# loro-dev/loro

Hardware: NVIDIA H100
Metric: merged CRDT ops/sec (batched docs) (higher is better)
Workload: dtype int64

## Files before the change

loro_b200/csrc/engine.cu:

```cuda
#include "../../include/loro_b200.h"

#include <algorithm>
#include <atomic>
#include <chrono>
#include <memory>
#include <mutex>
#include <string>
#include <thread>
#include <unordered_map>
#include <vector>
#include <cstring>
#include <cstdio>
#include <cstdlib>
#include <sched.h>

#include "lb_defs.h"
#include "k_frame.cuh"
#include "k_decode.cuh"
#include "k_decode_warp.cuh"
#include "k_resolve.cuh"
#include "k_classify.cuh"
#include "k_checkout.cuh"
#include "k_seq.cuh"
#include "k_tree.cuh"
// ... 322 lines not shown
struct DocsetBlob { std::shared_ptr<DocsetBuf> buf; u64 off; u32 len; };
struct DocsetDoc { std::vector<DocsetBlob> blobs; };
struct lb_docset {
    int device = 0;
    std::mutex mu;
    std::unordered_map<u64, DocsetDoc> docs;
    u64 stored_bytes = 0;
};

struct lb_exports {
    struct Answer { lb_status status; const char* error; const uint8_t* bytes; size_t len; };
    std::vector<Answer> answers;
    std::vector<std::unique_ptr<uint8_t[]>> bufs;
};

namespace {

const int TPB = 128;
inline unsigned nblk(u64 n, int tpb = TPB) { return (unsigned)((n + tpb - 1) / tpb); }

#define LB_BATCH_LAUNCH(b, kernel, grid, block, smem, ...)                          \
    do {                                                                            \
        LB_LAUNCH(kernel, grid, block, smem, (b)->dev.stream, __VA_ARGS__);         \
        (b)->timings.kernel_launches++;                                             \
    } while (0)

u32* BatchTables::* const SG_TABLES[] = {
    &BatchTables::sg_src, &BatchTables::sg_r0, &BatchTables::sg_from, &BatchTables::sg_atoms, &BatchTables::sg_est,
    &BatchTables::sg_nmops, &BatchTables::sg_ndel, &BatchTables::sg_nrows, &BatchTables::sg_last_head, &BatchTables::sg_skip};
u32* BatchTables::* const FC_TABLES[] = {
    &BatchTables::fc_src, &BatchTables::fc_pos, &BatchTables::fc_r0, &BatchTables::fc_from, &BatchTables::fc_atoms,
    &BatchTables::fc_nrows, &BatchTables::fc_ndel, &BatchTables::fc_skip, &BatchTables::fc_tail, &BatchTables::fc_est};

void launch_exp_encode(lb_batch* b, u64 NOB, const BatchTables& xt, XBlock* xb, u32* xscratch, u8* out, int retry, bool cuts) {
    if (!NOB) return;
    const bool capped = NOB >= LB_XENC_BOUNDED_MIN_BLOCKS;
    if (cuts && capped) LB_BATCH_LAUNCH(b, k_exp_encode_cut<1>, nblk(NOB, 64), 64, 0, b->d_docs, NOB, xt, xb, xscratch, out, retry);
    else if (cuts) LB_BATCH_LAUNCH(b, k_exp_encode_cut<0>, nblk(NOB, 64), 64, 0, b->d_docs, NOB, xt, xb, xscratch, out, retry);
    else if (capped) LB_BATCH_LAUNCH(b, k_exp_encode<1>, nblk(NOB, 64), 64, 0, b->d_docs, NOB, xt, xb, xscratch, out, retry);
    else LB_BATCH_LAUNCH(b, k_exp_encode<0>, nblk(NOB, 64), 64, 0, b->d_docs, NOB, xt, xb, xscratch, out, retry);
}

unsigned seq_resident_ctas(int device) {
#ifdef LB_SIMT_EMU
    (void)device;
    return 1;
#else
    static std::atomic<unsigned> ctas[64];
    std::atomic<unsigned>& n = ctas[(unsigned)device % 64];
    if (!n.load(std::memory_order_relaxed)) {
        int per_sm = 0, sms = 0;
        CK(cudaOccupancyMaxActiveBlocksPerMultiprocessor(&per_sm, k_seq_integrate<1>, 32 * LB_SEQ_WARPS, 0));
        CK(cudaDeviceGetAttribute(&sms, cudaDevAttrMultiProcessorCount, device));
        if (per_sm < 1 || sms < 1) {
            g_last_error = "k_seq_integrate: no CTA fits a multiprocessor";
            throw lb_status(LB_ERR_CUDA);
        }
        n.store((unsigned)per_sm * (unsigned)sms, std::memory_order_relaxed);
    }
    return n.load(std::memory_order_relaxed);
#endif
}

void trace_point(lb_batch* b, const char* name);
void mark(lb_batch* b, BatchEvent e) {
    CK(cudaEventRecord(b->ev[e], b->dev.stream));
    b->ev_recorded[e] = true;
}

template <class T>
T d2h_one(lb_batch* b, const T* src) {
    T v;
    CK(cudaMemcpyAsync(&v, src, sizeof(T), cudaMemcpyDeviceToHost, b->dev.stream));
// ... 1433 lines not shown
```

loro_b200/csrc/k_export.cuh:

```cuda
#pragma once
#include "lb_tables.cuh"

enum { XK_NONE = 0, XK_LIST = 1, XK_TEXT = 2, XK_DEL = 3, XK_MAPSET = 4, XK_MAPDEL = 5, XK_TREE = 6 };
#define LB_MAX_BLOCK_SIZE 4096
#define XF_HEAD 1u
#define XF_SEG 2u

struct XDoc {
    u32 n_fc, n_mb;
    u32 flags;
    u32 n_prank;
    u64 ob0;
    u64 scratch0;
    u64 exp_off;
    u32 exp_len;
    u32 scratch_words;
    u64 stage0;
    u64 ovf0;
    u64 restage0;
};
struct XBlock {
    u32 doc;
    u32 fc0, fc1;
    u32 len;
    u32 sec_len[8];
    u32 col_len[9];
    u64 off;
    u64 scratch;
    u32 n_rows, n_dels;
    u32 n_ops, n_del_ops, n_pos;
    u64 stage;
    u32 stage_cap;
    u32 ovf;
};

struct XSink {
    u8* dst;
    u64 n, cap;
    __device__ __forceinline__ XSink(u8* d, u64 c) : dst(d), n(0), cap(c) {}
    __device__ __forceinline__ void put(u8 c) { if (n < cap) dst[n] = c; n++; }
    __device__ __forceinline__ void varint(u64 v) { while (v >= 0x80) { put((u8)(v | 0x80)); v >>= 7; } put((u8)v); }
    __device__ __forceinline__ void zigzag(i64 v) { varint(((u64)v << 1) ^ (u64)(v >> 63)); }
    __device__ __forceinline__ void copy(const u8* s, u64 len) {
        if (n + len <= cap) {
            u8* d = dst + n;
            u64 i = 0;
            while (i < len && ((uintptr_t)(d + i) & 3)) { d[i] = s[i]; i++; }
            for (; i + 4 <= len; i += 4) {
                u32 w = (u32)s[i] | ((u32)s[i + 1] << 8) | ((u32)s[i + 2] << 16) | ((u32)s[i + 3] << 24);
                *(u32*)(d + i) = w;
            }
            for (; i < len; i++) d[i] = s[i];
        }
        n += len;
    }
};
__device__ __forceinline__ u32 varint_len(u64 v) { u32 k = 1; while (v >= 0x80) { v >>= 7; k++; } return k; }

struct XOp {
    u8 xk; u32 cidx; i32 ctr; u32 atoms; i32 prop; u32 f0, f1; i32 f2; u32 st0, nst;
    u32 g;
};
__device__ __forceinline__ u32 xop_estimate(const XOp& o) {
    switch (o.xk) {
        case XK_LIST: return 4 * o.atoms;
        case XK_TEXT: return o.f1 - o.f0;
        case XK_DEL: return 8;
        case XK_TREE: return 8;
        default: return 3;
    }
}
__device__ __forceinline__ u32 str_gen(u32 end) {
    u32 k = 0;
    u64 cap = 32;
    while (cap < end) { cap <<= 1; k++; }
    return k;
}
__device__ __forceinline__ bool d_bidi(const XOp& o) { return o.f2 == 1 || o.f2 == -1; }
__device__ __forceinline__ i64 d_start_pos(const XOp& o) { return o.f2 > 0 ? o.prop : (i64)o.prop + 1 + o.f2; }
__device__ __forceinline__ i64 d_next_pos(const XOp& o) { return o.f2 > 0 ? d_start_pos(o) : d_start_pos(o) - 1; }
__device__ __forceinline__ i64 d_prev_pos(const XOp& o) { return o.f2 > 0 ? o.prop : (i64)o.prop + 1; }
__device__ __forceinline__ i64 d_id_end(const XOp& o) { return (i64)(i32)o.f1 + (o.f2 < 0 ? -o.f2 : o.f2); }
__device__ inline bool xop_mergable(const XOp& a, const XOp& b) {
    if (a.ctr + (i32)a.atoms != b.ctr || a.cidx != b.cidx || a.xk != b.xk) return false;
    switch (a.xk) {
        case XK_LIST: return (i64)a.prop + a.atoms == b.prop && a.f1 == b.f0;
        case XK_TEXT: return (i64)a.prop + a.atoms == b.prop && a.f1 == b.f0 && a.g == b.g;
// ... 439 lines not shown

struct XEntry {
    u32 src, from;
    u32 pos, r0;
    u32 atoms, est_ops, nmops, ndel, nrows;
    u32 skip;
    u32 tail;
    u32 lh_ch, lh_row;
    XOp last;
    bool last_valid;
};
struct XStore {
    bool have_block, open_valid, open_starts_block;
    u32 blk_est;
    XEntry open;
    XOp back;
};
__device__ __forceinline__ bool xmsg_same(const BatchTables& t, u32 a, u32 b) {
    u32 la = t.ch_msg_len[a], lb = t.ch_msg_len[b];
    if (la != lb) return false;
    const u8* pa = t.bytes + t.ch_msg_off[a];
    const u8* pb = t.bytes + t.ch_msg_off[b];
    for (u32 i = 0; i < la; i++)
        if (pa[i] != pb[i]) return false;
    return true;
}
__device__ __forceinline__ u32 xentry_ndeps(const BatchTables& t, const XEntry& e) {
    return e.from ? 1u : t.ch_ndeps[e.src] + (t.ch_dep_self[e.src] ? 1u : 0u);
}
struct XRows {
    const BatchTables& t; u32 pos; u32 r; u32 ch; u32 nr; u64 row0;
    u32 skip;
    __device__ XRows(const BatchTables& t_, u32 pos_, u32 r_) : t(t_), pos(pos_), r(r_), skip(0) { load(); }
    __device__ void load() { ch = t.ch_aorder[pos]; change_rows(t, ch, &row0, &nr); }
    __device__ u64 row() const { return row0 + r; }
    __device__ void next() {
        r++;
        skip = 0;
        while (r >= nr) {
            pos++; r = 0; ch = t.ch_aorder[pos];
            if (!t.ch_applied[ch]) { nr = 0; continue; }
            change_rows(t, ch, &row0, &nr);
            if (t.ch_trim[ch]) { r = t.sg_r0[ch]; skip = t.sg_skip[ch]; }
        }
    }
};
__device__ inline XOp xop_gather(const BatchTables& t, const DocInfo& di, XRows& it, u32& left, u32 skip = 0, u32 tail = 0) {
    XOp o = xop_from_row(t, di, it.ch, it.row());
    if (skip) xop_slice_front(t, o, it.row(), skip);
    left--;
    if (left) it.next();
    while (left && !(xr_flag(t, it.row()) & XF_HEAD)) {
        XOp x = xop_from_row(t, di, it.ch, it.row());
        if (it.skip) xop_slice_front(t, x, it.row(), it.skip);
        xop_merge(o, x);
        left--;
        if (left) it.next();
    }
    if (!left && tail) xop_slice_back(t, o, it.row(), tail);
    return o;
}
__device__ inline XOp xentry_last_op(const BatchTables& t, const DocInfo& di, const XEntry& E) {
    if (E.last_valid) return E.last;
    u64 row0;
    u32 nr;
    change_rows(t, E.lh_ch, &row0, &nr);
// ... 363 lines not shown
    {
        i64 prev_delta = 0;
        for (u32 i = 1; i < n; i++) {
            i64 dl = val(i) - val(i - 1);
            i64 x = dl - prev_delta;
            prev_delta = dl;
            if (x == 0) total_bits += 1;
            else if (x >= -63 && x <= 64) total_bits += 9;
            else if (x >= -255 && x <= 256) total_bits += 12;
            else if (x >= -2047 && x <= 2048) total_bits += 16;
            else if (x >= -1048575 && x <= 1048576) total_bits += 26;
            else total_bits += 69;
        }
    }
    int used = (int)(total_bits & 7);
    s.put((u8)(used == 0 ? 8 : used));
    XBits bw(s);
    i64 prev_delta = 0;
    for (u32 i = 1; i < n; i++) {
        i64 dl = val(i) - val(i - 1);
        i64 x = dl - prev_delta;
        prev_delta = dl;
        if (x == 0) bw.bit(false);
        else if (x >= -63 && x <= 64) { bw.bits(2, 2); bw.bits((u64)(x + 63), 7); }
        else if (x >= -255 && x <= 256) { bw.bits(6, 3); bw.bits((u64)(x + 255), 9); }
        else if (x >= -2047 && x <= 2048) { bw.bits(14, 4); bw.bits((u64)(x + 2047), 12); }
        else if (x >= -1048575 && x <= 1048576) { bw.bits(30, 5); bw.bits((u64)(x + 1048575), 21); }
        else { bw.bits(31, 5); bw.bits((u64)x, 64); }
    }
    if (bw.nbits) s.put((u8)((bw.cur & 0xFF) << (8 - bw.nbits)));
}

struct XReg {
    u32* ord; u32* inv; u32 n;
    __device__ u32 reg(u32 v) {
        if (inv[v] != 0xFFFFFFFFu) return inv[v];
        inv[v] = n;
        ord[n] = v;
        return n++;
    }
};
__device__ inline void xvalue_copy(XSink& s, const u8* p, u32 n, const BatchTables& t, u64 src_key0, XReg& keys) {
    Cur c(p, n);
    u32 stack[24];
    int sp = 0;
    while (!c.err) {
        while (sp > 0 && (stack[sp - 1] & 0x7fffffffu) == 0) sp--;
        if (sp == 0 && c.empty()) return;
        if (sp > 0) {
            stack[sp - 1]--;
            if (stack[sp - 1] & 0x80000000u) {
                u32 dk = t.key_map[src_key0 + (u32)c.varint()];
                s.varint(keys.reg(dk));
            }
        }
        u8 kind = c.get();
        s.put(kind);
        switch (kind) {
            case 0: case 1: case 2: break;
            case 3: { const u8* a = c.p; (void)c.sleb(); s.copy(a, (u64)(c.p - a)); break; }
            case 4: { const u8* a = c.p; c.skip(8); s.copy(a, (u64)(c.p - a)); break; }
            case 5: case 6: { const u8* a = c.p; u64 l = c.varint(); c.skip(l); s.copy(a, (u64)(c.p - a)); break; }
            case 7: case 8: {
                u64 cnt = c.varint();
                s.varint(cnt);
                if (sp >= 24 || cnt > (1u << 28)) return;
                stack[sp++] = (u32)cnt | (kind == 8 ? 0x80000000u : 0u);
                break;
            }
            case 9: s.put(c.get()); break;
            default: return;
        }
    }
// ... 40 lines not shown
    const DocInfo& di = docs[d];
    if (di.code != DOC_OK || !di.has_tree) return;
    const u64 p_lo = t.blocks[di.b0].pos0;
    const u32 n = (u32)(t.blocks[di.b1].pos0 - p_lo);
    u64* key = t.ps_key + p_lo;
    u32* val = t.ps_val + p_lo;
    for (u32 i = lane; i < n; i += 32) {
        const u8* pb = t.pos_pool + t.pos_off[p_lo + i];
        u32 pl = t.pos_len[p_lo + i];
        u64 k = 0;
        for (u32 q = 0; q < 8; q++) k = (k << 8) | (q < pl ? pb[q] : 0u);
        if (k == ~0ull) k--;
        key[i] = k;
        val[i] = i;
    }
    __syncwarp();
    warp_sort_pairs(key, val, n, lane, [&](u32 a, u32 b) -> bool { return xpos_cmp(t, (u32)p_lo + a, (u32)p_lo + b) < 0; });
    u32 carry = 0;
    for (u32 j0 = 0; j0 < n; j0 += 32) {
        u32 j = j0 + (u32)lane;
        int fresh = 0;
        if (j < n) fresh = (j == 0 || xpos_cmp(t, (u32)p_lo + val[j - 1], (u32)p_lo + val[j]) != 0) ? 1 : 0;
        int incl = warp_incl_scan(fresh, lane);
        if (j < n) {
            u32 rank = carry + (u32)incl - 1;
            t.pos_rank[p_lo + val[j]] = rank;
            if (fresh) t.pos_rep[p_lo + rank] = (u32)p_lo + val[j];
        }
        carry += (u32)__shfl_sync(LB_FULL, incl, 31);
    }
    if (lane == 0) t.xdoc[d].n_prank = carry;
}

#define LB_XENC_BOUNDED_MIN_BLOCKS 100000ull
template <int CUT>
__device__ __forceinline__ void exp_encode_body(
    const DocInfo* __restrict__ docs, u64 n_blocks, const BatchTables& t, XBlock* __restrict__ xb,
                             u32* __restrict__ scratch, u8* __restrict__ out, int retry) {
    u64 bi_ = (u64)blockIdx.x * blockDim.x + threadIdx.x;
    if (bi_ >= n_blocks) return;
    XBlock B = xb[bi_];
    if (retry) {
        if (!B.ovf) return;
        out += t.xdoc[B.doc].restage0;
    }
    const DocInfo& di = docs[B.doc];
    const u32 P = di.P, K = di.K, C = di.C;
    u32* sc = scratch + B.scratch;
    XReg peers, keys, cids;
    peers.ord = sc; peers.inv = sc + P;
    keys.ord = sc + 2 * P; keys.inv = keys.ord + K;
    cids.ord = keys.ord + 2 * K; cids.inv = cids.ord + C;
    u32* c_cidx = cids.ord + 2 * C;
    u32* c_prop = c_cidx + B.n_rows;
    u32* c_vt = c_prop + B.n_rows;
    u32* c_atoms = c_vt + B.n_rows;
    u32* d_peer = c_atoms + B.n_rows;
    u32* d_ctr = d_peer + B.n_dels;
    u32* d_len = d_ctr + B.n_dels;
    const bool has_tree = (t.xdoc[B.doc].flags & 2u) != 0;
    const bool has_maps = (t.xdoc[B.doc].flags & 4u) != 0;
    u32* p_rank = d_len + B.n_dels;
    const u64 pos_lo = has_tree ? t.blocks[di.b0].pos0 : 0;
    auto pos_local = [&](u32 gpos) -> u32 {
        u32 r = t.pos_rank[gpos];
        u32 lo = 0, hi = B.n_pos;
        while (lo < hi) { u32 mid = (lo + hi) >> 1; if (p_rank[mid] < r) lo = mid + 1; else hi = mid; }
        return lo;
    };
    auto w_tree_value = [&](XSink& s, u32 ti) {
        uint4 ids = t.tr_ids[ti];
        u32 pk = ids.z & 3u;
        s.varint(peers.inv[ids.x]);
        s.varint(ids.y);
        s.varint(pk == TRP_DELETED ? 0u : pos_local(t.tr_pos[ti]));
        s.put(pk == TRP_ROOT ? 1 : 0);
        if (pk != TRP_ROOT) { s.varint(peers.inv[ids.z >> 2]); s.varint(ids.w); }
    };
    const u32 fc0 = B.fc0, N = B.fc1 - B.fc0;
    const u32 first_src = t.fc_src[fc0];
    u32 n_dep = 0;
    for (u32 j = 0; j < N; j++) n_dep += t.fc_from[fc0 + j] ? 0u : t.ch_ndeps[t.fc_src[fc0 + j]];
    for (u32 i = 0; i < P; i++) peers.inv[i] = 0xFFFFFFFFu;
    for (u32 i = 0; i < K; i++) keys.inv[i] = 0xFFFFFFFFu;
    for (u32 i = 0; i < C; i++) cids.inv[i] = 0xFFFFFFFFu;
    peers.n = keys.n = cids.n = 0;
    peers.reg(t.peer_map[t.blocks[t.ch_block[first_src]].peer0]);
    B.n_pos = 0;
    if (has_tree) {
        u32 m = 0;
        for (u32 j = 0; j < N; j++) {
            XRows it(t, t.fc_pos[fc0 + j], t.fc_r0[fc0 + j]);
            u32 left = t.fc_nrows[fc0 + j];
            while (left) {
                uint4 r = xr_rec(t, it.row());
                if ((r.x & 7u) == XK_TREE && t.tr_pos[r.w] != 0xFFFFFFFFu) p_rank[m++] = t.pos_rank[t.tr_pos[r.w]];
                left--;
                if (left) it.next();
            }
        }
        auto sift = [&](u32 root, u32 end) {
            while (true) {
                u32 c = 2 * root + 1;
                if (c >= end) break;
                if (c + 1 < end && p_rank[c + 1] > p_rank[c]) c++;
                if (p_rank[root] >= p_rank[c]) break;
                u32 tmp = p_rank[root]; p_rank[root] = p_rank[c]; p_rank[c] = tmp;
                root = c;
            }
        };
        for (u32 i = m / 2; i-- > 0;) sift(i, m);
        for (u32 e = m; e-- > 1;) { u32 tmp = p_rank[0]; p_rank[0] = p_rank[e]; p_rank[e] = tmp; sift(0, e); }
        u32 w = 0;
        for (u32 i = 0; i < m; i++) if (i == 0 || p_rank[i] != p_rank[w - 1]) p_rank[w++] = p_rank[i];
        B.n_pos = w;
    }
    XSink vs(out + B.stage, B.stage_cap);
    u32 n_ops = 0, n_del = 0;
    u32 prev_cidx = 0, prev_prop = 0, prev_dp = 0, prev_dc = 0, prev_dl = 0;
    for (u32 j = 0; j < N; j++) {
        XRows it(t, t.fc_pos[fc0 + j], t.fc_r0[fc0 + j]);
        u32 left = t.fc_nrows[fc0 + j];
        u32 skip = t.fc_skip[fc0 + j];
        while (left) {
            XRows it0 = it;
            const u32 left0 = left;
            const u32 skip0 = skip;
            XOp o = xop_gather(t, di, it, left, skip);
            if (CUT && !left) xop_slice_back(t, o, it.row(), t.fc_tail[fc0 + j]);
            skip = left ? it.skip : 0u;
            if (o.xk == XK_LIST) { vs.put(7); vs.varint(o.atoms); }
            else if (o.xk == XK_TEXT) vs.varint(o.f1 - o.f0);
            u32 lc = cids.reg(o.cidx);
            u32 lp = (o.xk == XK_MAPSET || o.xk == XK_MAPDEL) ? keys.reg((u32)o.prop) : (u32)o.prop;
            if (o.xk == XK_LIST || o.xk == XK_TEXT || o.xk == XK_MAPSET) {
                u32 k = left0 - left;
                while (k) {
                    const u8* pp;
                    u32 pn;
                    const u32 sk = k == left0 - left ? skip0 : it0.skip;
                    xr_payload_skip(t, it0.row(), o.xk, sk, &pp, &pn);
                    if (CUT && k == 1 && !left && t.fc_tail[fc0 + j]) xr_payload_drop_tail(o.xk, xr_len(t, it0.row()) - sk, t.fc_tail[fc0 + j], pp, &pn);
                    if (has_maps && o.xk != XK_TEXT) xvalue_copy(vs, pp, pn, t, t.blocks[t.ch_block[it0.ch]].key0, keys);
                    else vs.copy(pp, pn);
                    k--;
                    if (k) it0.next();
                }
            }
            c_cidx[n_ops] = lc - prev_cidx; prev_cidx = lc;
            c_prop[n_ops] = lp - prev_prop; prev_prop = lp;
            c_vt[n_ops] = xk_value_type(o.xk);
            c_atoms[n_ops] = o.atoms;
            if (o.xk == XK_TREE) {
                uint4 ids = t.tr_ids[o.f0];
                peers.reg(ids.x);
                if ((ids.z & 3u) != TRP_ROOT) peers.reg(ids.z >> 2);
                w_tree_value(vs, o.f0);
            }
            if (o.xk == XK_DEL) {
                u32 dp = peers.reg(o.f0);
                d_peer[n_del] = dp - prev_dp; prev_dp = dp;
                d_ctr[n_del] = o.f1 - prev_dc; prev_dc = o.f1;
                d_len[n_del] = (u32)o.f2 - prev_dl; prev_dl = (u32)o.f2;
                n_del++;
            }
            n_ops++;
        }
    }
    B.n_ops = n_ops;
    B.n_del_ops = n_del;
    B.sec_len[7] = (u32)vs.n;
    for (u32 i = 0; i < cids.n; i++) {
        const DocContainer& dc = t.dcont[di.cid0 + cids.ord[i]];
        if (dc.is_root) keys.reg(dc.key_or_peer); else peers.reg(dc.key_or_peer);
    }
    for (u32 j = 0; j < N; j++) {
        if (t.fc_from[fc0 + j]) continue;
        u32 src = t.fc_src[fc0 + j];
        const BlockInfo& sb = t.blocks[t.ch_block[src]];
        for (u32 k = 0; k < t.ch_ndeps[src]; k++) peers.reg(t.peer_map[sb.peer0 + t.dep_peer_idx[t.ch_dep0[src] + k]]);
    }

    auto dep_self = [&](u32 j) -> bool { return t.fc_from[fc0 + j] ? true : t.ch_dep_self[t.fc_src[fc0 + j]] != 0; };
    auto dep_local = [&](XDeps& dc, u32 i) -> i64 {
        u64 di_ = dc.at(i);
        const BlockInfo& sb = t.blocks[t.ch_block[t.fc_src[fc0 + dc.j]]];
        return (i64)peers.inv[t.peer_map[sb.peer0 + t.dep_peer_idx[di_]]];
    };
    auto lamport = [&](u32 j) -> i64 { return (i64)t.ch_lamport[t.fc_src[fc0 + j]] + t.fc_from[fc0 + j]; };
    auto w_header = [&](XSink& s) {
        s.varint(peers.n);
        for (u32 i = 0; i < peers.n; i++) {
            u64 id = t.dpeer[di.peer0 + peers.ord[i]].id;
            for (int k = 0; k < 8; k++) s.put((u8)(id >> (8 * k)));
        }
        for (u32 j = 0; j + 1 < N; j++) s.varint(t.fc_atoms[fc0 + j]);
        enc_boolrle(s, N, dep_self);
        { XDeps dc(t, fc0, N); enc_anyrle(s, N, [&](u32 j) -> i64 { return (i64)dc.nd(j); }, WrVarint()); }
        { XDeps dc(t, fc0, N); enc_anyrle(s, n_dep, [&](u32 i) -> i64 { return dep_local(dc, i); }, WrVarint()); }
        { XDeps dc(t, fc0, N); enc_dod(s, n_dep, [&](u32 i) -> i64 { return (i64)t.dep_counter[dc.at(i)]; }); }
        enc_dod(s, N - 1, lamport);
    };
    auto w_meta = [&](XSink& s) {
        enc_dod(s, N, [&](u32 j) -> i64 { return t.ch_ts[t.fc_src[fc0 + j]]; });
        enc_anyrle(s, N, [&](u32 j) -> i64 { return (i64)t.ch_msg_len[t.fc_src[fc0 + j]]; }, WrVarint());
        for (u32 j = 0; j < N; j++) {
            u32 src = t.fc_src[fc0 + j];
            s.copy(t.bytes + t.ch_msg_off[src], t.ch_msg_len[src]);
        }
    };
    auto w_cids = [&](XSink& s) {
        s.varint(cids.n);
        for (u32 i = 0; i < cids.n; i++) {
            const DocContainer& dc = t.dcont[di.cid0 + cids.ord[i]];
            s.varint(4);
            s.put(dc.is_root ? 1 : 0);
            s.put(dc.type);
            if (dc.is_root) { s.varint(0); s.zigzag((i64)keys.inv[dc.key_or_peer]); }
            else { s.varint(peers.inv[dc.key_or_peer]); s.zigzag((i64)dc.counter); }
        }
    };
    auto w_keys = [&](XSink& s) {
        for (u32 i = 0; i < keys.n; i++) {
            u32 k = keys.ord[i];
            s.varint(t.dkey_len[di.key0 + k]);
            s.copy(t.bytes + t.dkey_off[di.key0 + k], t.dkey_len[di.key0 + k]);
        }
    };
    auto w_opcol = [&](XSink& s, int col) {
        switch (col) {
            case 0: enc_anyrle(s, n_ops, [&](u32 i) -> i64 { return (i64)(i32)c_cidx[i]; }, WrZigzag()); break;
            case 1: enc_anyrle(s, n_ops, [&](u32 i) -> i64 { return (i64)(i32)c_prop[i]; }, WrZigzag()); break;
            case 2: enc_anyrle(s, n_ops, [&](u32 i) -> i64 { return (i64)c_vt[i]; }, WrByte()); break;
            default: enc_anyrle(s, n_ops, [&](u32 i) -> i64 { return (i64)c_atoms[i]; }, WrVarint());
        }
    };
    auto w_delcol = [&](XSink& s, int col) {
        switch (col) {
            case 0: enc_anyrle(s, n_del, [&](u32 i) -> i64 { return (i64)(i32)d_peer[i]; }, WrZigzag()); break;
            case 1: enc_anyrle(s, n_del, [&](u32 i) -> i64 { return (i64)(i32)d_ctr[i]; }, WrZigzag()); break;
            default: enc_anyrle(s, n_del, [&](u32 i) -> i64 { return (i64)(i32)d_len[i]; }, WrZigzag());
        }
    };
    auto pos_bytes_of = [&](u32 i, const u8** pb) -> u32 { u32 g = t.pos_rep[pos_lo + p_rank[i]]; *pb = t.pos_pool + t.pos_off[g]; return t.pos_len[g]; };
    auto pos_common = [&](u32 i) -> u32 {
        if (i == 0) return 0;
        const u8 *a, *b;
        u32 la = pos_bytes_of(i - 1, &a), lb = pos_bytes_of(i, &b);
        u32 n = la < lb ? la : lb, k = 0;
        while (k < n && a[k] == b[k]) k++;
        return k;
    };
    auto w_poscol = [&](XSink& s, int col) {
        if (col == 0) enc_anyrle(s, B.n_pos, [&](u32 i) -> i64 { return (i64)pos_common(i); }, WrVarint());
        else {
            s.varint(B.n_pos);
            for (u32 i = 0; i < B.n_pos; i++) {
                const u8* pb;
                u32 pl = pos_bytes_of(i, &pb), c = pos_common(i);
                s.varint(pl - c);
                s.copy(pb + c, pl - c);
            }
        }
    };
    u32 counter_len = 0;
    for (u32 j = 0; j < N; j++) counter_len += t.fc_atoms[fc0 + j];
    u32 counter0 = (u32)t.ch_counter[first_src] + t.fc_from[fc0];
    u32 lam0 = (u32)lamport(0);
    u32 lam_len = (u32)lamport(N - 1) + t.fc_atoms[B.fc1 - 1] - lam0;
    XSink s(out + B.stage, B.stage_cap);
    s.n = B.sec_len[7];
    s.varint(counter0);
    s.varint(counter_len);
    s.varint(lam0);
    s.varint(lam_len);
    s.varint(N);
    u64 m = s.n;
    w_header(s); B.sec_len[0] = (u32)(s.n - m); m = s.n;
    w_meta(s); B.sec_len[1] = (u32)(s.n - m); m = s.n;
    w_cids(s); B.sec_len[2] = (u32)(s.n - m); m = s.n;
    w_keys(s); B.sec_len[3] = (u32)(s.n - m); m = s.n;
    u32 tot = 0;
    if (B.n_pos) {
        tot = 2;
        for (int c = 0; c < 2; c++) { w_poscol(s, c); B.col_len[7 + c] = (u32)(s.n - m); m = s.n; tot += varint_len(B.col_len[7 + c]) + B.col_len[7 + c]; }
    }
    B.sec_len[4] = tot;
    tot = 2;
    for (int c = 0; c < 4; c++) { w_opcol(s, c); B.col_len[c] = (u32)(s.n - m); m = s.n; tot += varint_len(B.col_len[c]) + B.col_len[c]; }
    B.sec_len[5] = tot;
    if (n_del) {
        tot = 2;
        for (int c = 0; c < 3; c++) { w_delcol(s, c); B.col_len[4 + c] = (u32)(s.n - m); m = s.n; tot += varint_len(B.col_len[4 + c]) + B.col_len[4 + c]; }
        B.sec_len[6] = tot;
    } else B.sec_len[6] = 0;
    B.ovf |= s.n > s.cap;
    u32 len = varint_len(counter0) + varint_len(counter_len) + varint_len(lam0) + varint_len(lam_len) + varint_len(N);
    for (int i = 0; i < 8; i++) len += varint_len(B.sec_len[i]) + B.sec_len[i];
    B.len = len;
    xb[bi_] = B;
}

template <int CAPPED> __global__ void k_exp_encode(const DocInfo* __restrict__ docs, u64 n_blocks, const __grid_constant__ BatchTables t, XBlock* __restrict__ xb,
                                                 u32* __restrict__ scratch, u8* __restrict__ out, int retry);
template <> __global__ void k_exp_encode<0>(const DocInfo* __restrict__ docs, u64 n_blocks, const __grid_constant__ BatchTables t, XBlock* __restrict__ xb,
                                            u32* __restrict__ scratch, u8* __restrict__ out, int retry) {
    exp_encode_body<0>(docs, n_blocks, t, xb, scratch, out, retry);
}
template <> __global__ void __launch_bounds__(64, 5) k_exp_encode<1>(const DocInfo* __restrict__ docs, u64 n_blocks, const __grid_constant__ BatchTables t,
                                                                     XBlock* __restrict__ xb, u32* __restrict__ scratch,
                                                                     u8* __restrict__ out, int retry) {
    exp_encode_body<0>(docs, n_blocks, t, xb, scratch, out, retry);
}
template <int CAPPED> __global__ void k_exp_encode_cut(const DocInfo* __restrict__ docs, u64 n_blocks, const __grid_constant__ BatchTables t, XBlock* __restrict__ xb,
                                                     u32* __restrict__ scratch, u8* __restrict__ out, int retry);
template <> __global__ void k_exp_encode_cut<0>(const DocInfo* __restrict__ docs, u64 n_blocks, const __grid_constant__ BatchTables t, XBlock* __restrict__ xb,
                                                u32* __restrict__ scratch, u8* __restrict__ out, int retry) {
    exp_encode_body<1>(docs, n_blocks, t, xb, scratch, out, retry);
}
template <> __global__ void __launch_bounds__(64, 5) k_exp_encode_cut<1>(const DocInfo* __restrict__ docs, u64 n_blocks, const __grid_constant__ BatchTables t,
                                                                         XBlock* __restrict__ xb, u32* __restrict__ scratch,
                                                                         u8* __restrict__ out, int retry) {
    exp_encode_body<1>(docs, n_blocks, t, xb, scratch, out, retry);
}

__global__ void k_exp_layout(const DocInfo* __restrict__ docs, u32 n_docs, const __grid_constant__ BatchTables t, XBlock* __restrict__ xb,
                             u32* __restrict__ padded_len, u32* __restrict__ n_ovf, u32* __restrict__ n_restage) {
    u32 d = blockIdx.x * blockDim.x + threadIdx.x;
    if (d >= n_docs) return;
    XDoc& x = t.xdoc[d];
    u32 len = 0, ovf = 0, restage = 0;
    if (docs[d].code == DOC_OK && !(x.flags & 1) && (!t.x_req || t.x_req[d])) {
        len = 22;
        for (u32 i = 0; i < x.n_mb; i++) {
            XBlock& b = xb[x.ob0 + i];
            len += varint_len(b.len);
            b.off = len;
            len += b.len;
            if (b.ovf) {
                ovf++;
                b.stage = restage;
                b.stage_cap = b.len;
                restage += b.len;
            }
        }
    }
    x.exp_len = len;
    padded_len[d] = (len + 15u) & ~15u;
    n_ovf[d] = ovf;
    n_restage[d] = restage;
}

__global__ void k_exp_finish(const DocInfo* __restrict__ docs, u32 n_docs, const __grid_constant__ BatchTables t, const XBlock* __restrict__ xb,
                             const u8* __restrict__ stage, const u8* __restrict__ restage, u8* __restrict__ out) {
    u32 d = (blockIdx.x * blockDim.x + threadIdx.x) >> 5;
    int lane = threadIdx.x & 31;
    if (d >= n_docs) return;
    const XDoc& x = t.xdoc[d];
    if (x.exp_len == 0) return;
    u8* b = out + x.exp_off;
    for (u32 i = 0; i < x.n_mb; i++) {
        const XBlock& B = xb[x.ob0 + i];
        u8* dst = b + B.off - varint_len(B.len);
        const u8* src = (B.ovf ? restage + x.restage0 : stage) + B.stage;
        u64 o = 0, so = B.sec_len[7];
        auto prefix = [&](u32 v) {
            if (lane == 0) { XSink s(dst + o, ~0ull); s.varint(v); }
            o += varint_len(v);
        };
        auto piece = [&](u32 n) {
            u8* dd = dst + o;
            const u8* ss = src + so;
            u32 k = (u32)lane;
            for (; k + 96 < n; k += 128) {
                u8 a = ss[k], c = ss[k + 32], e = ss[k + 64], g = ss[k + 96];
                dd[k] = a; dd[k + 32] = c; dd[k + 64] = e; dd[k + 96] = g;
            }
            for (; k < n; k += 32) dd[k] = ss[k];
            o += n;
            so += n;
        };
        u32 head = B.len;
        for (int k = 0; k < 8; k++) head -= varint_len(B.sec_len[k]) + B.sec_len[k];
        prefix(B.len);
        piece(head);
        for (int k = 0; k < 4; k++) { prefix(B.sec_len[k]); piece(B.sec_len[k]); }
        prefix(B.sec_len[4]);
        if (B.n_pos) {
            prefix(1); prefix(2);
            for (int c = 0; c < 2; c++) { prefix(B.col_len[7 + c]); piece(B.col_len[7 + c]); }
        }
        prefix(B.sec_len[5]);
        prefix(1); prefix(4);
        for (int c = 0; c < 4; c++) { prefix(B.col_len[c]); piece(B.col_len[c]); }
        prefix(B.sec_len[6]);
        if (B.n_del_ops) {
            prefix(1); prefix(3);
            for (int c = 0; c < 3; c++) { prefix(B.col_len[4 + c]); piece(B.col_len[4 + c]); }
        }
        prefix(B.sec_len[7]);
// ... 14 lines not shown
```

Baseline: 427.8 million.

## Reduce register pressure in export encoder and use grid-stride launch

The export encode kernel now writes XBlock fields in place rather than copying the whole struct into registers, and it keeps scratch offsets as u32 indices instead of many pointers. It also narrows XSink counters to 32 bits and folds the column encoders into one indexed path. The launch becomes a grid-stride loop with the grid capped at a per-SM multiple, and every variant gets launch bounds of 64 threads with 10 minimum blocks. The aim is lower register use and higher occupancy. The risks are more global-memory traffic from in-place field writes, spills forced by the tighter launch bounds, and 32-bit overflow of sink offsets on very large blocks.

```diff
diff --git a/loro_b200/csrc/engine.cu b/loro_b200/csrc/engine.cu
--- a/loro_b200/csrc/engine.cu
+++ b/loro_b200/csrc/engine.cu
@@ -378,13 +378,29 @@
     &BatchTables::fc_src, &BatchTables::fc_pos, &BatchTables::fc_r0, &BatchTables::fc_from, &BatchTables::fc_atoms,
     &BatchTables::fc_nrows, &BatchTables::fc_ndel, &BatchTables::fc_skip, &BatchTables::fc_tail, &BatchTables::fc_est};
 
+unsigned device_sms(int device) {
+#ifdef LB_SIMT_EMU
+    (void)device;
+    return 1;
+#else
+    static std::atomic<unsigned> sms[64];
+    std::atomic<unsigned>& n = sms[(unsigned)device % 64];
+    if (!n.load(std::memory_order_relaxed)) {
+        int v = 0;
+        CK(cudaDeviceGetAttribute(&v, cudaDevAttrMultiProcessorCount, device));
+        n.store(v > 0 ? (unsigned)v : 1u, std::memory_order_relaxed);
+    }
+    return n.load(std::memory_order_relaxed);
+#endif
+}
+
 void launch_exp_encode(lb_batch* b, u64 NOB, const BatchTables& xt, XBlock* xb, u32* xscratch, u8* out, int retry, bool cuts) {
     if (!NOB) return;
-    const bool capped = NOB >= LB_XENC_BOUNDED_MIN_BLOCKS;
-    if (cuts && capped) LB_BATCH_LAUNCH(b, k_exp_encode_cut<1>, nblk(NOB, 64), 64, 0, b->d_docs, NOB, xt, xb, xscratch, out, retry);
-    else if (cuts) LB_BATCH_LAUNCH(b, k_exp_encode_cut<0>, nblk(NOB, 64), 64, 0, b->d_docs, NOB, xt, xb, xscratch, out, retry);
-    else if (capped) LB_BATCH_LAUNCH(b, k_exp_encode<1>, nblk(NOB, 64), 64, 0, b->d_docs, NOB, xt, xb, xscratch, out, retry);
-    else LB_BATCH_LAUNCH(b, k_exp_encode<0>, nblk(NOB, 64), 64, 0, b->d_docs, NOB, xt, xb, xscratch, out, retry);
+    const u64 sms = device_sms(b->device);
+    unsigned grid = nblk(NOB, 64);
+    if (grid > LB_XENC_MIN_CTAS * sms) grid = (unsigned)(LB_XENC_CTAS_PER_SM * sms);
+    if (cuts) LB_BATCH_LAUNCH(b, k_exp_encode_cut<0>, grid, 64, 0, b->d_docs, NOB, xt, xb, xscratch, out, retry);
+    else LB_BATCH_LAUNCH(b, k_exp_encode<0>, grid, 64, 0, b->d_docs, NOB, xt, xb, xscratch, out, retry);
 }
 
 unsigned seq_resident_ctas(int device) {
diff --git a/loro_b200/csrc/k_export.cuh b/loro_b200/csrc/k_export.cuh
--- a/loro_b200/csrc/k_export.cuh
+++ b/loro_b200/csrc/k_export.cuh
@@ -36,8 +36,8 @@
 
 struct XSink {
     u8* dst;
-    u64 n, cap;
-    __device__ __forceinline__ XSink(u8* d, u64 c) : dst(d), n(0), cap(c) {}
+    u32 n, cap;
+    __device__ __forceinline__ XSink(u8* d, u32 c) : dst(d), n(0), cap(c) {}
     __device__ __forceinline__ void put(u8 c) { if (n < cap) dst[n] = c; n++; }
     __device__ __forceinline__ void varint(u64 v) { while (v >= 0x80) { put((u8)(v | 0x80)); v >>= 7; } put((u8)v); }
     __device__ __forceinline__ void zigzag(i64 v) { varint(((u64)v << 1) ^ (u64)(v >> 63)); }
@@ -52,7 +52,7 @@
             }
             for (; i < len; i++) d[i] = s[i];
         }
-        n += len;
+        n += (u32)len;
     }
 };
 __device__ __forceinline__ u32 varint_len(u64 v) { u32 k = 1; while (v >= 0x80) { v >>= 7; k++; } return k; }
@@ -558,6 +558,11 @@
     const BatchTables& t; u32 pos; u32 r; u32 ch; u32 nr; u64 row0;
     u32 skip;
     __device__ XRows(const BatchTables& t_, u32 pos_, u32 r_) : t(t_), pos(pos_), r(r_), skip(0) { load(); }
+    XRows(const XRows&) = default;
+    __device__ XRows& operator=(const XRows& o) {
+        pos = o.pos; r = o.r; ch = o.ch; nr = o.nr; row0 = o.row0; skip = o.skip;
+        return *this;
+    }
     __device__ void load() { ch = t.ch_aorder[pos]; change_rows(t, ch, &row0, &nr); }
     __device__ u64 row() const { return row0 + r; }
     __device__ void next() {
@@ -987,13 +992,19 @@
 }
 
 struct XReg {
-    u32* ord; u32* inv; u32 n;
+    u32* sc; u32 ord, inv, n;
+    __device__ XReg(u32* sc_, u32 ord_, u32 cap) : sc(sc_), ord(ord_), inv(ord_ + cap), n(0) {
+        for (u32 i = 0; i < cap; i++) sc[inv + i] = 0xFFFFFFFFu;
+    }
     __device__ u32 reg(u32 v) {
-        if (inv[v] != 0xFFFFFFFFu) return inv[v];
-        inv[v] = n;
-        ord[n] = v;
+        const u32 r = sc[inv + v];
+        if (r != 0xFFFFFFFFu) return r;
+        sc[inv + v] = n;
+        sc[ord + n] = v;
         return n++;
     }
+    __device__ u32 at(u32 i) const { return sc[ord + i]; }
+    __device__ u32 local(u32 v) const { return sc[inv + v]; }
 };
 __device__ inline void xvalue_copy(XSink& s, const u8* p, u32 n, const BatchTables& t, u64 src_key0, XReg& keys) {
     Cur c(p, n);
@@ -1100,61 +1111,35 @@
     if (lane == 0) t.xdoc[d].n_prank = carry;
 }
 
-#define LB_XENC_BOUNDED_MIN_BLOCKS 100000ull
 template <int CUT>
-__device__ __forceinline__ void exp_encode_body(
-    const DocInfo* __restrict__ docs, u64 n_blocks, const BatchTables& t, XBlock* __restrict__ xb,
-                             u32* __restrict__ scratch, u8* __restrict__ out, int retry) {
-    u64 bi_ = (u64)blockIdx.x * blockDim.x + threadIdx.x;
-    if (bi_ >= n_blocks) return;
-    XBlock B = xb[bi_];
+__device__ __forceinline__ void exp_encode_body(const DocInfo* __restrict__ docs, u64 bi_, const BatchTables& t, XBlock* __restrict__ xb,
+                                                u32* __restrict__ scratch, u8* __restrict__ out, int retry) {
+    XBlock& B = xb[bi_];
+    const u32 doc = B.doc;
     if (retry) {
         if (!B.ovf) return;
-        out += t.xdoc[B.doc].restage0;
-    }
-    const DocInfo& di = docs[B.doc];
+        out += t.xdoc[doc].restage0;
+    }
+    const DocInfo& di = docs[doc];
+    const u32 fc0 = B.fc0, N = B.fc1 - fc0;
+    const u32 n_rows = B.n_rows, n_dels = B.n_dels;
+    u32* sc = scratch + B.scratch;
     const u32 P = di.P, K = di.K, C = di.C;
-    u32* sc = scratch + B.scratch;
-    XReg peers, keys, cids;
-    peers.ord = sc; peers.inv = sc + P;
-    keys.ord = sc + 2 * P; keys.inv = keys.ord + K;
-    cids.ord = keys.ord + 2 * K; cids.inv = cids.ord + C;
-    u32* c_cidx = cids.ord + 2 * C;
-    u32* c_prop = c_cidx + B.n_rows;
-    u32* c_vt = c_prop + B.n_rows;
-    u32* c_atoms = c_vt + B.n_rows;
-    u32* d_peer = c_atoms + B.n_rows;
-    u32* d_ctr = d_peer + B.n_dels;
-    u32* d_len = d_ctr + B.n_dels;
-    const bool has_tree = (t.xdoc[B.doc].flags & 2u) != 0;
-    const bool has_maps = (t.xdoc[B.doc].flags & 4u) != 0;
-    u32* p_rank = d_len + B.n_dels;
+    XReg peers(sc, 0, P), keys(sc, 2 * P, K), cids(sc, 2 * P + 2 * K, C);
+    const u32 o_col = 2 * (P + K + C), o_del = o_col + 4 * n_rows, o_rank = o_del + 3 * n_dels;
+    const bool has_tree = (t.xdoc[doc].flags & 2u) != 0;
     const u64 pos_lo = has_tree ? t.blocks[di.b0].pos0 : 0;
+    u32 n_pos = 0, n_ops = 0, n_del = 0, vlen;
     auto pos_local = [&](u32 gpos) -> u32 {
         u32 r = t.pos_rank[gpos];
-        u32 lo = 0, hi = B.n_pos;
-        while (lo < hi) { u32 mid = (lo + hi) >> 1; if (p_rank[mid] < r) lo = mid + 1; else hi = mid; }
+        u32 lo = 0, hi = n_pos;
+        while (lo < hi) { u32 mid = (lo + hi) >> 1; if (sc[o_rank + mid] < r) lo = mid + 1; else hi = mid; }
         return lo;
     };
-    auto w_tree_value = [&](XSink& s, u32 ti) {
-        uint4 ids = t.tr_ids[ti];
-        u32 pk = ids.z & 3u;
-        s.varint(peers.inv[ids.x]);
-        s.varint(ids.y);
-        s.varint(pk == TRP_DELETED ? 0u : pos_local(t.tr_pos[ti]));
-        s.put(pk == TRP_ROOT ? 1 : 0);
-        if (pk != TRP_ROOT) { s.varint(peers.inv[ids.z >> 2]); s.varint(ids.w); }
-    };
-    const u32 fc0 = B.fc0, N = B.fc1 - B.fc0;
-    const u32 first_src = t.fc_src[fc0];
-    u32 n_dep = 0;
-    for (u32 j = 0; j < N; j++) n_dep += t.fc_from[fc0 + j] ? 0u : t.ch_ndeps[t.fc_src[fc0 + j]];
-    for (u32 i = 0; i < P; i++) peers.inv[i] = 0xFFFFFFFFu;
-    for (u32 i = 0; i < K; i++) keys.inv[i] = 0xFFFFFFFFu;
-    for (u32 i = 0; i < C; i++) cids.inv[i] = 0xFFFFFFFFu;
-    peers.n = keys.n = cids.n = 0;
-    peers.reg(t.peer_map[t.blocks[t.ch_block[first_src]].peer0]);
-    B.n_pos = 0;
+    {
+    const bool has_maps = (t.xdoc[doc].flags & 4u) != 0;
+    u32* p_rank = sc + o_rank;
+    peers.reg(t.peer_map[t.blocks[t.ch_block[t.fc_src[fc0]]].peer0]);
     if (has_tree) {
         u32 m = 0;
         for (u32 j = 0; j < N; j++) {
@@ -1181,10 +1166,9 @@
         for (u32 e = m; e-- > 1;) { u32 tmp = p_rank[0]; p_rank[0] = p_rank[e]; p_rank[e] = tmp; sift(0, e); }
         u32 w = 0;
         for (u32 i = 0; i < m; i++) if (i == 0 || p_rank[i] != p_rank[w - 1]) p_rank[w++] = p_rank[i];
-        B.n_pos = w;
+        n_pos = w;
     }
     XSink vs(out + B.stage, B.stage_cap);
-    u32 n_ops = 0, n_del = 0;
     u32 prev_cidx = 0, prev_prop = 0, prev_dp = 0, prev_dc = 0, prev_dl = 0;
     for (u32 j = 0; j < N; j++) {
         XRows it(t, t.fc_pos[fc0 + j], t.fc_r0[fc0 + j]);
@@ -1201,45 +1185,49 @@
             else if (o.xk == XK_TEXT) vs.varint(o.f1 - o.f0);
             u32 lc = cids.reg(o.cidx);
             u32 lp = (o.xk == XK_MAPSET || o.xk == XK_MAPDEL) ? keys.reg((u32)o.prop) : (u32)o.prop;
+            sc[o_col + n_ops] = lc - prev_cidx; prev_cidx = lc;
+            sc[o_col + n_rows + n_ops] = lp - prev_prop; prev_prop = lp;
+            sc[o_col + 2 * n_rows + n_ops] = xk_value_type(o.xk);
+            sc[o_col + 3 * n_rows + n_ops] = o.atoms;
+            if (o.xk == XK_TREE) {
+                uint4 ids = t.tr_ids[o.f0];
+                const u32 pk = ids.z & 3u;
+                vs.varint(peers.reg(ids.x));
+                if (pk != TRP_ROOT) peers.reg(ids.z >> 2);
+                vs.varint(ids.y);
+                vs.varint(pk == TRP_DELETED ? 0u : pos_local(t.tr_pos[o.f0]));
+                vs.put(pk == TRP_ROOT ? 1 : 0);
+                if (pk != TRP_ROOT) { vs.varint(peers.local(ids.z >> 2)); vs.varint(ids.w); }
+            }
+            if (o.xk == XK_DEL) {
+                u32 dp = peers.reg(o.f0);
+                sc[o_del + n_del] = dp - prev_dp; prev_dp = dp;
+                sc[o_del + n_dels + n_del] = o.f1 - prev_dc; prev_dc = o.f1;
+                sc[o_del + 2 * n_dels + n_del] = (u32)o.f2 - prev_dl; prev_dl = (u32)o.f2;
+                n_del++;
+            }
+            n_ops++;
             if (o.xk == XK_LIST || o.xk == XK_TEXT || o.xk == XK_MAPSET) {
+                it = it0;
                 u32 k = left0 - left;
                 while (k) {
                     const u8* pp;
                     u32 pn;
-                    const u32 sk = k == left0 - left ? skip0 : it0.skip;
-                    xr_payload_skip(t, it0.row(), o.xk, sk, &pp, &pn);
-                    if (CUT && k == 1 && !left && t.fc_tail[fc0 + j]) xr_payload_drop_tail(o.xk, xr_len(t, it0.row()) - sk, t.fc_tail[fc0 + j], pp, &pn);
-                    if (has_maps && o.xk != XK_TEXT) xvalue_copy(vs, pp, pn, t, t.blocks[t.ch_block[it0.ch]].key0, keys);
+                    const u32 sk = k == left0 - left ? skip0 : it.skip;
+                    xr_payload_skip(t, it.row(), o.xk, sk, &pp, &pn);
+                    if (CUT && k == 1 && !left && t.fc_tail[fc0 + j]) xr_payload_drop_tail(o.xk, xr_len(t, it.row()) - sk, t.fc_tail[fc0 + j], pp, &pn);
+                    if (has_maps && o.xk != XK_TEXT) xvalue_copy(vs, pp, pn, t, t.blocks[t.ch_block[it.ch]].key0, keys);
                     else vs.copy(pp, pn);
                     k--;
-                    if (k) it0.next();
+                    if (k) it.next();
                 }
-            }
-            c_cidx[n_ops] = lc - prev_cidx; prev_cidx = lc;
-            c_prop[n_ops] = lp - prev_prop; prev_prop = lp;
-            c_vt[n_ops] = xk_value_type(o.xk);
-            c_atoms[n_ops] = o.atoms;
-            if (o.xk == XK_TREE) {
-                uint4 ids = t.tr_ids[o.f0];
-                peers.reg(ids.x);
-                if ((ids.z & 3u) != TRP_ROOT) peers.reg(ids.z >> 2);
-                w_tree_value(vs, o.f0);
-            }
-            if (o.xk == XK_DEL) {
-                u32 dp = peers.reg(o.f0);
-                d_peer[n_del] = dp - prev_dp; prev_dp = dp;
-                d_ctr[n_del] = o.f1 - prev_dc; prev_dc = o.f1;
-                d_len[n_del] = (u32)o.f2 - prev_dl; prev_dl = (u32)o.f2;
-                n_del++;
-            }
-            n_ops++;
-        }
-    }
-    B.n_ops = n_ops;
-    B.n_del_ops = n_del;
-    B.sec_len[7] = (u32)vs.n;
+                if (left) it.next();
+            }
+        }
+    }
+    vlen = vs.n;
     for (u32 i = 0; i < cids.n; i++) {
-        const DocContainer& dc = t.dcont[di.cid0 + cids.ord[i]];
+        const DocContainer& dc = t.dcont[di.cid0 + cids.at(i)];
         if (dc.is_root) keys.reg(dc.key_or_peer); else peers.reg(dc.key_or_peer);
     }
     for (u32 j = 0; j < N; j++) {
@@ -1248,18 +1236,25 @@
         const BlockInfo& sb = t.blocks[t.ch_block[src]];
         for (u32 k = 0; k < t.ch_ndeps[src]; k++) peers.reg(t.peer_map[sb.peer0 + t.dep_peer_idx[t.ch_dep0[src] + k]]);
     }
-
+    }
+    B.n_pos = n_pos;
+    B.n_ops = n_ops;
+    B.n_del_ops = n_del;
+    B.sec_len[7] = vlen;
+
+    u32 n_dep = 0;
+    for (u32 j = 0; j < N; j++) n_dep += t.fc_from[fc0 + j] ? 0u : t.ch_ndeps[t.fc_src[fc0 + j]];
     auto dep_self = [&](u32 j) -> bool { return t.fc_from[fc0 + j] ? true : t.ch_dep_self[t.fc_src[fc0 + j]] != 0; };
     auto dep_local = [&](XDeps& dc, u32 i) -> i64 {
         u64 di_ = dc.at(i);
         const BlockInfo& sb = t.blocks[t.ch_block[t.fc_src[fc0 + dc.j]]];
-        return (i64)peers.inv[t.peer_map[sb.peer0 + t.dep_peer_idx[di_]]];
+        return (i64)peers.local(t.peer_map[sb.peer0 + t.dep_peer_idx[di_]]);
     };
     auto lamport = [&](u32 j) -> i64 { return (i64)t.ch_lamport[t.fc_src[fc0 + j]] + t.fc_from[fc0 + j]; };
     auto w_header = [&](XSink& s) {
         s.varint(peers.n);
         for (u32 i = 0; i < peers.n; i++) {
-            u64 id = t.dpeer[di.peer0 + peers.ord[i]].id;
+            u64 id = t.dpeer[di.peer0 + peers.at(i)].id;
             for (int k = 0; k < 8; k++) s.put((u8)(id >> (8 * k)));
         }
         for (u32 j = 0; j + 1 < N; j++) s.varint(t.fc_atoms[fc0 + j]);
@@ -1280,37 +1275,34 @@
     auto w_cids = [&](XSink& s) {
         s.varint(cids.n);
         for (u32 i = 0; i < cids.n; i++) {
-            const DocContainer& dc = t.dcont[di.cid0 + cids.ord[i]];
+            const DocContainer& dc = t.dcont[di.cid0 + cids.at(i)];
             s.varint(4);
             s.put(dc.is_root ? 1 : 0);
             s.put(dc.type);
-            if (dc.is_root) { s.varint(0); s.zigzag((i64)keys.inv[dc.key_or_peer]); }
-            else { s.varint(peers.inv[dc.key_or_peer]); s.zigzag((i64)dc.counter); }
+            if (dc.is_root) { s.varint(0); s.zigzag((i64)keys.local(dc.key_or_peer)); }
+            else { s.varint(peers.local(dc.key_or_peer)); s.zigzag((i64)dc.counter); }
         }
     };
     auto w_keys = [&](XSink& s) {
         for (u32 i = 0; i < keys.n; i++) {
-            u32 k = keys.ord[i];
+            u32 k = keys.at(i);
             s.varint(t.dkey_len[di.key0 + k]);
             s.copy(t.bytes + t.dkey_off[di.key0 + k], t.dkey_len[di.key0 + k]);
         }
     };
     auto w_opcol = [&](XSink& s, int col) {
+        const u32* c = sc + o_col + col * n_rows;
         switch (col) {
-            case 0: enc_anyrle(s, n_ops, [&](u32 i) -> i64 { return (i64)(i32)c_cidx[i]; }, WrZigzag()); break;
-            case 1: enc_anyrle(s, n_ops, [&](u32 i) -> i64 { return (i64)(i32)c_prop[i]; }, WrZigzag()); break;
-            case 2: enc_anyrle(s, n_ops, [&](u32 i) -> i64 { return (i64)c_vt[i]; }, WrByte()); break;
-            default: enc_anyrle(s, n_ops, [&](u32 i) -> i64 { return (i64)c_atoms[i]; }, WrVarint());
+            case 0: case 1: enc_anyrle(s, n_ops, [&](u32 i) -> i64 { return (i64)(i32)c[i]; }, WrZigzag()); break;
+            case 2: enc_anyrle(s, n_ops, [&](u32 i) -> i64 { return (i64)c[i]; }, WrByte()); break;
+            default: enc_anyrle(s, n_ops, [&](u32 i) -> i64 { return (i64)c[i]; }, WrVarint());
         }
     };
     auto w_delcol = [&](XSink& s, int col) {
-        switch (col) {
-            case 0: enc_anyrle(s, n_del, [&](u32 i) -> i64 { return (i64)(i32)d_peer[i]; }, WrZigzag()); break;
-            case 1: enc_anyrle(s, n_del, [&](u32 i) -> i64 { return (i64)(i32)d_ctr[i]; }, WrZigzag()); break;
-            default: enc_anyrle(s, n_del, [&](u32 i) -> i64 { return (i64)(i32)d_len[i]; }, WrZigzag());
-        }
+        const u32* c = sc + o_del + col * n_dels;
+        enc_anyrle(s, n_del, [&](u32 i) -> i64 { return (i64)(i32)c[i]; }, WrZigzag());
     };
-    auto pos_bytes_of = [&](u32 i, const u8** pb) -> u32 { u32 g = t.pos_rep[pos_lo + p_rank[i]]; *pb = t.pos_pool + t.pos_off[g]; return t.pos_len[g]; };
+    auto pos_bytes_of = [&](u32 i, const u8** pb) -> u32 { u32 g = t.pos_rep[pos_lo + sc[o_rank + i]]; *pb = t.pos_pool + t.pos_off[g]; return t.pos_len[g]; };
     auto pos_common = [&](u32 i) -> u32 {
         if (i == 0) return 0;
         const u8 *a, *b;
@@ -1320,10 +1312,10 @@
         return k;
     };
     auto w_poscol = [&](XSink& s, int col) {
-        if (col == 0) enc_anyrle(s, B.n_pos, [&](u32 i) -> i64 { return (i64)pos_common(i); }, WrVarint());
+        if (col == 0) enc_anyrle(s, n_pos, [&](u32 i) -> i64 { return (i64)pos_common(i); }, WrVarint());
         else {
-            s.varint(B.n_pos);
-            for (u32 i = 0; i < B.n_pos; i++) {
+            s.varint(n_pos);
+            for (u32 i = 0; i < n_pos; i++) {
                 const u8* pb;
                 u32 pl = pos_bytes_of(i, &pb), c = pos_common(i);
                 s.varint(pl - c);
@@ -1331,65 +1323,59 @@
             }
         }
     };
+    const u32 first_src = t.fc_src[fc0];
     u32 counter_len = 0;
     for (u32 j = 0; j < N; j++) counter_len += t.fc_atoms[fc0 + j];
     u32 counter0 = (u32)t.ch_counter[first_src] + t.fc_from[fc0];
     u32 lam0 = (u32)lamport(0);
-    u32 lam_len = (u32)lamport(N - 1) + t.fc_atoms[B.fc1 - 1] - lam0;
+    u32 lam_len = (u32)lamport(N - 1) + t.fc_atoms[fc0 + N - 1] - lam0;
     XSink s(out + B.stage, B.stage_cap);
-    s.n = B.sec_len[7];
+    s.n = vlen;
     s.varint(counter0);
     s.varint(counter_len);
     s.varint(lam0);
     s.varint(lam_len);
     s.varint(N);
-    u64 m = s.n;
-    w_header(s); B.sec_len[0] = (u32)(s.n - m); m = s.n;
-    w_meta(s); B.sec_len[1] = (u32)(s.n - m); m = s.n;
-    w_cids(s); B.sec_len[2] = (u32)(s.n - m); m = s.n;
-    w_keys(s); B.sec_len[3] = (u32)(s.n - m); m = s.n;
+    u32 len = s.n - vlen;
+    auto section = [&](int i, u32 n) { B.sec_len[i] = n; len += varint_len(n) + n; };
+    section(7, vlen);
+    u32 m = s.n;
+    w_header(s); section(0, s.n - m); m = s.n;
+    w_meta(s); section(1, s.n - m); m = s.n;
+    w_cids(s); section(2, s.n - m); m = s.n;
+    w_keys(s); section(3, s.n - m); m = s.n;
     u32 tot = 0;
-    if (B.n_pos) {
+    if (n_pos) {
         tot = 2;
-        for (int c = 0; c < 2; c++) { w_poscol(s, c); B.col_len[7 + c] = (u32)(s.n - m); m = s.n; tot += varint_len(B.col_len[7 + c]) + B.col_len[7 + c]; }
-    }
-    B.sec_len[4] = tot;
+        for (int c = 0; c < 2; c++) { w_poscol(s, c); const u32 l = s.n - m; B.col_len[7 + c] = l; m = s.n; tot += varint_len(l) + l; }
+    }
+    section(4, tot);
     tot = 2;
-    for (int c = 0; c < 4; c++) { w_opcol(s, c); B.col_len[c] = (u32)(s.n - m); m = s.n; tot += varint_len(B.col_len[c]) + B.col_len[c]; }
-    B.sec_len[5] = tot;
+    for (int c = 0; c < 4; c++) { w_opcol(s, c); const u32 l = s.n - m; B.col_len[c] = l; m = s.n; tot += varint_len(l) + l; }
+    section(5, tot);
+    tot = 0;
     if (n_del) {
         tot = 2;
-        for (int c = 0; c < 3; c++) { w_delcol(s, c); B.col_len[4 + c] = (u32)(s.n - m); m = s.n; tot += varint_len(B.col_len[4 + c]) + B.col_len[4 + c]; }
-        B.sec_len[6] = tot;
-    } else B.sec_len[6] = 0;
-    B.ovf |= s.n > s.cap;
-    u32 len = varint_len(counter0) + varint_len(counter_len) + varint_len(lam0) + varint_len(lam_len) + varint_len(N);
-    for (int i = 0; i < 8; i++) len += varint_len(B.sec_len[i]) + B.sec_len[i];
+        for (int c = 0; c < 3; c++) { w_delcol(s, c); const u32 l = s.n - m; B.col_len[4 + c] = l; m = s.n; tot += varint_len(l) + l; }
+    }
+    section(6, tot);
+    if (s.n > s.cap) B.ovf = 1;
     B.len = len;
-    xb[bi_] = B;
-}
-
-template <int CAPPED> __global__ void k_exp_encode(const DocInfo* __restrict__ docs, u64 n_blocks, const __grid_constant__ BatchTables t, XBlock* __restrict__ xb,
-                                                 u32* __restrict__ scratch, u8* __restrict__ out, int retry);
-template <> __global__ void k_exp_encode<0>(const DocInfo* __restrict__ docs, u64 n_blocks, const __grid_constant__ BatchTables t, XBlock* __restrict__ xb,
-                                            u32* __restrict__ scratch, u8* __restrict__ out, int retry) {
-    exp_encode_body<0>(docs, n_blocks, t, xb, scratch, out, retry);
-}
-template <> __global__ void __launch_bounds__(64, 5) k_exp_encode<1>(const DocInfo* __restrict__ docs, u64 n_blocks, const __grid_constant__ BatchTables t,
-                                                                     XBlock* __restrict__ xb, u32* __restrict__ scratch,
-                                                                     u8* __restrict__ out, int retry) {
-    exp_encode_body<0>(docs, n_blocks, t, xb, scratch, out, retry);
-}
-template <int CAPPED> __global__ void k_exp_encode_cut(const DocInfo* __restrict__ docs, u64 n_blocks, const __grid_constant__ BatchTables t, XBlock* __restrict__ xb,
-                                                     u32* __restrict__ scratch, u8* __restrict__ out, int retry);
-template <> __global__ void k_exp_encode_cut<0>(const DocInfo* __restrict__ docs, u64 n_blocks, const __grid_constant__ BatchTables t, XBlock* __restrict__ xb,
-                                                u32* __restrict__ scratch, u8* __restrict__ out, int retry) {
-    exp_encode_body<1>(docs, n_blocks, t, xb, scratch, out, retry);
-}
-template <> __global__ void __launch_bounds__(64, 5) k_exp_encode_cut<1>(const DocInfo* __restrict__ docs, u64 n_blocks, const __grid_constant__ BatchTables t,
-                                                                         XBlock* __restrict__ xb, u32* __restrict__ scratch,
-                                                                         u8* __restrict__ out, int retry) {
-    exp_encode_body<1>(docs, n_blocks, t, xb, scratch, out, retry);
+}
+
+#define LB_XENC_MIN_CTAS 10
+#define LB_XENC_CTAS_PER_SM 6
+template <int V> __global__ void __launch_bounds__(64, LB_XENC_MIN_CTAS)
+k_exp_encode(const DocInfo* __restrict__ docs, u64 n_blocks, const __grid_constant__ BatchTables t, XBlock* __restrict__ xb,
+             u32* __restrict__ scratch, u8* __restrict__ out, int retry) {
+    for (u64 bi = (u64)blockIdx.x * blockDim.x + threadIdx.x; bi < n_blocks; bi += (u64)gridDim.x * blockDim.x)
+        exp_encode_body<0>(docs, bi, t, xb, scratch, out, retry);
+}
+template <int V> __global__ void __launch_bounds__(64, LB_XENC_MIN_CTAS)
+k_exp_encode_cut(const DocInfo* __restrict__ docs, u64 n_blocks, const __grid_constant__ BatchTables t, XBlock* __restrict__ xb,
+                 u32* __restrict__ scratch, u8* __restrict__ out, int retry) {
+    for (u64 bi = (u64)blockIdx.x * blockDim.x + threadIdx.x; bi < n_blocks; bi += (u64)gridDim.x * blockDim.x)
+        exp_encode_body<1>(docs, bi, t, xb, scratch, out, retry);
 }
 
 __global__ void k_exp_layout(const DocInfo* __restrict__ docs, u32 n_docs, const __grid_constant__ BatchTables t, XBlock* __restrict__ xb,
@@ -1433,7 +1419,7 @@
         const u8* src = (B.ovf ? restage + x.restage0 : stage) + B.stage;
         u64 o = 0, so = B.sec_len[7];
         auto prefix = [&](u32 v) {
-            if (lane == 0) { XSink s(dst + o, ~0ull); s.varint(v); }
+            if (lane == 0) { XSink s(dst + o, ~0u); s.varint(v); }
             o += varint_len(v);
         };
         auto piece = [&](u32 n) {
```

Result: faster. 434.3 million, median of 6 (+1.5%).
